# B10532021/Part-Aware_Measurement_for_3D_Pose_Estimation_and_Tracking

Hardware: AMD Instinct MI355X
Metric: multi-view frames/sec (end-to-end: HRNet-W48 2D pose + part-aware cross-view matching + DLT tracking) (higher is better)
Workload: dtype bf16 convs / f64 matching

## Files before the change

### part-aware_measurement_for_3d_pose_estimation_and_tracking_amd/csrc/pam_down.hip

```cpp
#include <hip/hip_runtime.h>
#include <stdint.h>
#include "../../include/pam.h"
#include "pam_resident.hpp"

namespace {

constexpr int PA = KStep48::PA, NST = KStep48::NST, WIMG = KStep48::WIMG;
constexpr int WPW = 6;
constexpr int BIASB = 2048;
constexpr int MTMAX = 3;
constexpr int D48_XSLOTS_MAX = (160 * 1024 - 2 * WIMG - BIASB) / PA;

struct D48Args {
    const uint16_t* in; const char* wpack; const float* bias; const uint16_t* res; uint16_t* out;
    int N, H, W, Ho, Wo, in_cs, out_cs, res_cs, relu, relu_from;
    int TR, TC, tiles_y, tiles_x, nitems, spw , xbytes;
    float inv_tc;
};

__device__ __attribute__((aligned(64))) const uint32_t g_d48_zero[16] = {0};

__global__ __launch_bounds__(512) void k_down48(D48Args a) {
    extern __shared__ __attribute__((aligned(1024))) char smem[];
    const int tid = threadIdx.x, lane = tid & 63, g = lane >> 4, l15 = lane & 15;
    const int wave = __builtin_amdgcn_readfirstlane(tid >> 6);
    const int bx = xcd_order(blockIdx.x, a.nitems);
    const int per_img = a.tiles_y * a.tiles_x;
    const int n = bx / per_img, trem = bx - n * per_img, tyi = trem / a.tiles_x, txi = trem - tyi * a.tiles_x;
    const int ty0 = tyi * a.TR, tx0 = txi * a.TC;
    const int NE = a.TC + 1, PWx = 2 * a.TC + 1, XR = 2 * a.TR + 1;
    const int slab0 = (int)blockIdx.y * a.spw;
    char* Xb = smem;
    float* bias_s = (float*)(smem + a.xbytes);
    char* Wb = smem + a.xbytes + BIASB;

    const float bv = (tid < a.spw * 48 && a.bias) ? a.bias[slab0 * 48 + tid] : 0.0f;
    const char* wsrc = a.wpack + (size_t)slab0 * WIMG + lane * 16;
    auto wdma = [&](int s) {
        char* dst = Wb + (s & 1) * WIMG;
#pragma unroll
        for (int k = 0; k < WPW; ++k) {
            const int p = min(wave + 8 * k, WIMG / 1024 - 1);
            __builtin_amdgcn_global_load_lds((glb_void*)(wsrc + (size_t)s * WIMG + p * 1024), (lds_void*)(dst + p * 1024), 16, 0, 0);
        }
    };
    wdma(0);
    {
        const int rowb = PWx * PA;
        const char* img = (const char*)a.in + (size_t)n * a.H * a.W * a.in_cs * 2;
        for (int k = 0; k * 1024 < rowb; ++k) {
            const int ob = k * 1024 + lane * 16;
            const int q = (int)(((unsigned)ob * 43691u) >> 22);
            const int rem = ob - q * PA;
            const int c = q < NE ? 2 * q : 2 * (q - NE) + 1;
            const int ix = 2 * tx0 - 1 + c;
            const bool okx = ob < rowb && (unsigned)ix < (unsigned)a.W;
            const long offx = (long)ix * a.in_cs * 2 + rem;
            if (ob < rowb) {
                for (int r = wave; r < XR; r += 8) {
                    const int iy = 2 * ty0 - 1 + r;
                    const bool ok = okx && (unsigned)iy < (unsigned)a.H;
                    const char* src = ok ? img + (size_t)iy * a.W * a.in_cs * 2 + offx : (const char*)g_d48_zero;
                    __builtin_amdgcn_global_load_lds((glb_void*)src, (lds_void*)(Xb + r * rowb + k * 1024), 16, 0, 0);
                }
            }
        }
    }
    if (tid < a.spw * 48) bias_s[tid] = bv;
    if (a.spw > 1) {
        wdma(1);
        asm volatile("s_waitcnt vmcnt(%0)" ::"n"(WPW) : "memory");
    } else {
        asm volatile("s_waitcnt vmcnt(0)" ::: "memory");
    }
    unsigned koff[NST];
#pragma unroll
    for (int st = 0; st < NST; ++st) {
        int k0 = 32 * st + 8 * g;
        if (k0 >= 432) k0 -= 16;
        const int t = k0 / 48, ch = k0 - 48 * t, ky = t / 3, kx = t - 3 * ky;
        koff[st] = (unsigned)((ky * PWx + (kx == 1 ? NE : (kx == 2 ? 1 : 0))) * PA + ch * 2);
    }
    const int npos = a.TR * a.TC;
    const int ntile = (npos + 15) >> 4, mt = (ntile - wave + 7) >> 3;
    const char* xl[MTMAX];
    long ooff[MTMAX];
#pragma unroll
    for (int i = 0; i < MTMAX; ++i) {
        const int m = (wave + 8 * i) * 16 + l15;
        const int r2 = fdiv_small(m, a.inv_tc), c2 = m - r2 * a.TC;
        const bool in_tile = m < npos;
        xl[i] = Xb + (in_tile ? (2 * r2 * PWx + c2) * PA : 0);
        const int oy = ty0 + r2, ox = tx0 + c2;
        ooff[i] = (in_tile && oy < a.Ho && ox < a.Wo) ? (long)(((size_t)n * a.Ho + oy) * a.Wo + ox) : -1;
    }
    const unsigned wlo = (unsigned)(l15 * 64 + ((g ^ KStep48::sigma(l15)) * 16));
    auto xaddr = [&](int i, int st) { return xl[i] + koff[st]; };

    asm volatile("s_barrier" ::: "memory");

    for (int s = 0; s < a.spw; ++s) {
        const int cb = (slab0 + s) * 48;
        u32x4 rq[MTMAX]; u32x2 rh[MTMAX];
        if (a.res) {
#pragma unroll
            for (int i = 0; i < MTMAX; ++i) {
                const uint16_t* rp = a.res + (ooff[i] >= 0 ? ooff[i] * a.res_cs + cb : 0);
                rq[i] = *(const u32x4*)(rp + 8 * g);
                rh[i] = *(const u32x2*)(rp + 32 + 4 * g);
            }
        }
        f32x4 acc[MTMAX][3];
        {
            const float* b = bias_s + s * 48;
            const f32x4 b0 = *(const f32x4*)(b + 8 * g), b1 = *(const f32x4*)(b + 8 * g + 4), b2 = *(const f32x4*)(b + 32 + 4 * g);
#pragma unroll
            for (int i = 0; i < MTMAX; ++i) { acc[i][0] = b0; acc[i][1] = b1; acc[i][2] = b2; }
        }
        const char* wl = Wb + (s & 1) * WIMG + wlo;
        if (mt >= 3) resident_pass<KStep48, 3>(acc, wl, xaddr, [](int) {});
        else if (mt == 2) resident_pass<KStep48, 2>(acc, wl, xaddr, [](int) {});
        else if (mt == 1) resident_pass<KStep48, 1>(acc, wl, xaddr, [](int) {});
        if (s + 1 < a.spw) {
            asm volatile("s_waitcnt vmcnt(0)" ::: "memory");
            asm volatile("s_barrier" ::: "memory");
            if (s + 2 < a.spw) wdma(s + 2);
        }
        const bool relu_lo = a.relu && cb + 8 * g >= a.relu_from, relu_hi = a.relu && cb + 32 + 4 * g >= a.relu_from;
#pragma unroll
        for (int i = 0; i < MTMAX; ++i) {
            if (i >= mt || ooff[i] < 0) continue;
            uint32_t ov[6];
#pragma unroll
            for (int j = 0; j < 3; ++j) {
                float v0 = acc[i][j][0], v1 = acc[i][j][1], v2 = acc[i][j][2], v3 = acc[i][j][3];
                if (a.res) {
                    const uint32_t r01 = j < 2 ? rq[i][2 * j] : rh[i][0], r23 = j < 2 ? rq[i][2 * j + 1] : rh[i][1];
                    v0 += bf16_lo(r01); v1 += bf16_hi(r01);
                    v2 += bf16_lo(r23); v3 += bf16_hi(r23);
                }
                ov[2 * j] = pack_bf16x2(v0, v1); ov[2 * j + 1] = pack_bf16x2(v2, v3);
                if (j < 2 ? relu_lo : relu_hi) { ov[2 * j] = relu_bf16x2(ov[2 * j]); ov[2 * j + 1] = relu_bf16x2(ov[2 * j + 1]); }
            }
            KStep48::store12(a.out + ooff[i] * a.out_cs + cb, g, ov);
        }
    }
}

bool d48_pick(int N, int Ho, int Wo, int nslab, int& TR, int& TC, int& G) {
    static thread_local int memo[8][7];
    static thread_local int memo_n = 0;
    for (int k = 0; k < 8 && k < memo_n; ++k)
        if (memo[k][0] == N && memo[k][1] == Ho && memo[k][2] == Wo && memo[k][3] == nslab) { TR = memo[k][4]; TC = memo[k][5]; G = memo[k][6]; return true; }
    long best = -1;
    for (int tr = 1; tr <= Ho; ++tr)
        for (int tc = 1; tc <= Wo; ++tc) {
            const int xs = (2 * tr + 1) * (2 * tc + 1), nt = (tr * tc + 15) / 16;
            if (xs > D48_XSLOTS_MAX || nt > 8 * MTMAX) continue;
            const long items = (long)N * ((Ho + tr - 1) / tr) * ((Wo + tc - 1) / tc);
            for (int gsz = 1; gsz <= nslab; ++gsz) {
                if (nslab % gsz) continue;
                const int spw = nslab / gsz;
                if (spw * 48 * 4 > BIASB) continue;
                const long fill = ((long)xs * PA + (long)spw * WIMG) / 24;
                const long mfma = (long)simd_tiles(nt, 0) * 3 * NST * 16 * spw;
                const long t = 5000 + (fill > mfma ? fill + mfma / 4 : mfma + fill / 4) + 500L * spw;
                const long wgs = items * gsz;
                const long cost = ((wgs + 255) / 256) * t * 4096 + wgs;
                if (best < 0 || cost < best) { best = cost; TR = tr; TC = tc; G = gsz; }
            }
        }
    if (best < 0) return false;
    int* m = memo[memo_n++ & 7];
    m[0] = N; m[1] = Ho; m[2] = Wo; m[3] = nslab; m[4] = TR; m[5] = TC; m[6] = G;
    return true;
}


struct DSArgs {
    const uint16_t* in; const uint16_t* wimg; const float* bias; uint16_t* out;
    int N, H, W, Ho, Wo, in_cs, Cout, TH, tiles_y, relu, relu_from;
    float inv_pwp, inv_wo;
};

template <int CIN, int NTW, int MT, int PMAX, int NBUF>
__global__ __launch_bounds__(512, 1) void k_down_s(DSArgs a) {
    constexpr int BN = 16 * NTW, NCHUNK = CIN / 32;
    constexpr int PIMG = PMAX * 64, WIMGS = 9 * BN * 64, BUF = PIMG + WIMGS;
    constexpr int PPW = PMAX / 64, WPIECES = WIMGS / 1024, WPWS = (WPIECES + 3) / 4, NPER = PPW + WPWS;
    static_assert(PMAX % 64 == 0 && WIMGS % 1024 == 0 && NPER * (NBUF - 1) <= 60 && NBUF >= 2 && NBUF <= 3, "ring shape");
    extern __shared__ __attribute__((aligned(1024))) char smem[];
    const int tid = threadIdx.x, lane = tid & 63, g = lane >> 4;
    const int wave = __builtin_amdgcn_readfirstlane(tid >> 6);
    const int ntiles = a.tiles_y * a.N;
    const int bx = xcd_order(blockIdx.x, ntiles);
    const int n = bx / a.tiles_y, ty0 = (bx - n * a.tiles_y) * a.TH;
    const int NEp = a.Wo + 1, PWp = 2 * a.Wo + 2, npatch = (2 * a.TH + 1) * PWp;
    const int npos = min(a.TH, a.Ho - ty0) * a.Wo;
    const int n0 = blockIdx.y * BN;

    if (wave >= 4) {
        const int lw = wave - 4;
        const char* psrc[PPW];
#pragma unroll
        for (int i = 0; i < PPW; ++i) {
            const int s = (lw + 4 * i) * 16 + (lane >> 2);
            const int gsrc = (lane & 3) ^ ((s >> 1) & 2);
            const int py = fdiv_small(s, a.inv_pwp), q = s - py * PWp;
            const int c = q < NEp ? 2 * q : 2 * (q - NEp) + 1;
            const int iy = 2 * ty0 - 1 + py, ix = c - 1;
            const bool ok = s < npatch && q <= 2 * a.Wo && (unsigned)iy < (unsigned)a.H && (unsigned)ix < (unsigned)a.W;
            psrc[i] = ok ? (const char*)a.in + (((size_t)n * a.H + iy) * a.W + ix) * (size_t)(a.in_cs * 2) + gsrc * 16 : (const char*)g_d48_zero;
        }
        const char* wsrc = (const char*)a.wimg + (size_t)blockIdx.y * NCHUNK * WIMGS + lane * 16;
        auto issue = [&](int c) {
            char* dst = smem + (size_t)((unsigned)c % (unsigned)NBUF) * BUF;
#pragma unroll
            for (int i = 0; i < (PPW > WPWS ? PPW : WPWS); ++i) {
                if (i < WPWS) {
                    const int j = min(lw + 4 * i, WPIECES - 1);
                    __builtin_amdgcn_global_load_lds((glb_void*)(wsrc + (size_t)c * WIMGS + j * 1024), (lds_void*)(dst + PIMG + j * 1024), 16, 0, 0);
                }
                if (i < PPW) {
                    const bool z = psrc[i] == (const char*)g_d48_zero;
                    __builtin_amdgcn_global_load_lds((glb_void*)(psrc[i] + (z ? 0 : c * 64)), (lds_void*)(dst + (lw + 4 * i) * 1024), 16, 0, 0);
                }
            }
        };
#pragma unroll
        for (int c = 0; c < NBUF - 1; ++c)
            if (c < NCHUNK) issue(c);
        for (int k = 0; k < NCHUNK; ++k) {
            const int fly = min(NCHUNK - 1 - k, NBUF - 2);
            dma_ring_wait<NPER, NBUF>(fly);
            asm volatile("s_barrier" ::: "memory");
            if (k + NBUF - 1 < NCHUNK) issue(k + NBUF - 1);
        }
        return;
    }

    f32x4 acc[MT][NTW];
    {
        f32x4 bias4[NTW];
#pragma unroll
        for (int j = 0; j < NTW; ++j) bias4[j] = a.bias ? *(const f32x4*)(a.bias + n0 + g * 4 * NTW + j * 4) : (f32x4){0.f, 0.f, 0.f, 0.f};
#pragma unroll
        for (int i = 0; i < MT; ++i)
#pragma unroll
            for (int j = 0; j < NTW; ++j) acc[i][j] = bias4[j];
    }
    unsigned aoff[MT][9];
    int opix[MT];
#pragma unroll
    for (int i = 0; i < MT; ++i) {
        const int m = (wave * MT + i) * 16 + (lane & 15);
        const int mm = m < npos ? m : 0;
        const int oy = fdiv_small(mm, a.inv_wo), ox = mm - oy * a.Wo;
        opix[i] = m < npos ? ((n * a.Ho + ty0 + oy) * a.Wo + ox) : -1;
#pragma unroll
        for (int t = 0; t < 9; ++t) {
            const int ky = t / 3, kx = t % 3;
            const int s = (2 * oy + ky) * PWp + ox + (kx == 1 ? NEp : (kx == 2 ? 1 : 0));
            aoff[i][t] = (unsigned)(s * 64 + ((g ^ ((s >> 1) & 2)) << 4));
        }
    }
    const unsigned woff = (unsigned)(PIMG + (lane & 15) * 64 + ((g ^ ((lane >> 1) & 2)) << 4));

    bf16x8 af[2][MT], bfr[2][NTW];
    auto ldfrag = [&](int k, int t, bf16x8* af_, bf16x8* bf_) {
        const char* buf = smem + (size_t)((unsigned)k % (unsigned)NBUF) * BUF;
#pragma unroll
        for (int j = 0; j < NTW; ++j) bf_[j] = *(const bf16x8*)(buf + woff + (t * BN + j * 16) * 64);
#pragma unroll
        for (int i = 0; i < MT; ++i) af_[i] = *(const bf16x8*)(buf + aoff[i][t]);
    };
    auto chunk = [&](int k, auto PARC) {
        constexpr int PAR = decltype(PARC)::value;
#pragma unroll
        for (int t = 0; t < 9; ++t) {
            const int cur = (t + PAR) & 1, nxt = cur ^ 1;
            if (t + 1 < 9) ldfrag(k, t + 1, af[nxt], bfr[nxt]);
            else if (k + 1 < NCHUNK) {
                __builtin_amdgcn_s_waitcnt(0xC07F);
                asm volatile("s_barrier" ::: "memory");
                ldfrag(k + 1, 0, af[nxt], bfr[nxt]);
            }
#pragma unroll
            for (int i = 0; i < MT; ++i)
#pragma unroll
                for (int j = 0; j < NTW; ++j)
                    acc[i][j] = __builtin_amdgcn_mfma_f32_16x16x32_bf16(__builtin_bit_cast(bf16x8_t, bfr[cur][j]),
                                                                       __builtin_bit_cast(bf16x8_t, af[cur][i]), acc[i][j], 0, 0, 0);
            spread<MT * NTW, MT + NTW>();
            __builtin_amdgcn_sched_barrier(0);
        }
    };
    asm volatile("s_barrier" ::: "memory");
    ldfrag(0, 0, af[0], bfr[0]);
    for (int k = 0; k < NCHUNK; k += 2) {
        chunk(k, std::integral_constant<int, 0>{});
        if (k + 1 < NCHUNK) chunk(k + 1, std::integral_constant<int, 1>{});
    }
#pragma unroll
    for (int i = 0; i < MT; ++i) {
        if (opix[i] < 0) continue;
        uint32_t ov[2 * NTW];
#pragma unroll
        for (int j = 0; j < NTW; ++j) {
            ov[2 * j] = pack_bf16x2(acc[i][j][0], acc[i][j][1]); ov[2 * j + 1] = pack_bf16x2(acc[i][j][2], acc[i][j][3]);
            if (a.relu && n0 + g * 4 * NTW + j * 4 >= a.relu_from) { ov[2 * j] = relu_bf16x2(ov[2 * j]); ov[2 * j + 1] = relu_bf16x2(ov[2 * j + 1]); }
        }
        row_store<NTW>(a.out + (size_t)opix[i] * a.Cout + n0 + g * 4 * NTW, g, ov);
    }
}

bool ds_pick(int Ho, int Wo, int Cin, int Cout, int& TH, int& bn) {
    if (Cin != 96 && Cin != 192) return false;
    bn = Cout % 64 == 0 ? 64 : (Cout % 48 == 0 ? 48 : 0);
    if (!bn) return false;
    const int PWp = 2 * Wo + 2;
    TH = 0;
    long best = 0;
    for (int t = Ho; t >= 1; --t) {
        if (t * Wo > 128 || (2 * t + 1) * PWp > 512) continue;
        const long cost = (Ho + t - 1) / t;
        if (TH == 0 || cost < best) { TH = t; best = cost; }
    }
    return TH >= 1;
}
template <int CIN, int NTW>
int launch_ds(hipStream_t s, const DSArgs& a) {
    constexpr int MT = 2, PMAX = 512, NBUF = 2;
    constexpr size_t lds = (size_t)NBUF * (PMAX * 64 + 9 * 16 * NTW * 64);
    static_assert(lds <= 160 * 1024, "LDS");
    if (!pam_max_dynamic_lds((const void*)k_down_s<CIN, NTW, MT, PMAX, NBUF>, (int)lds)) return PAM_E_HIP;
    pam_launch(k_down_s<CIN, NTW, MT, PMAX, NBUF>, dim3(a.tiles_y * a.N, a.Cout / (16 * NTW)), dim3(512), lds, s, a);
    return hipGetLastError() == hipSuccess ? PAM_OK : PAM_E_HIP;
}

}

extern "C" int pam_conv3x3s2_c48_tile(int N, int H, int W, int Cout, int32_t* out3) {
    if (N < 1 || H < 2 || W < 2 || Cout < 48 || Cout % 48 != 0 || !out3) return PAM_E_ARG;
    int tr = 0, tc = 0, gs = 0;
    if (!d48_pick(N, (H - 1) / 2 + 1, (W - 1) / 2 + 1, Cout / 48, tr, tc, gs)) return PAM_E_ARG;
    out3[0] = tr; out3[1] = tc; out3[2] = gs;
    return PAM_OK;
}

extern "C" int pam_conv3x3s2_c48_nhwc_bf16(void* stream, const void* in, int in_cstride, const void* wpack, const float* bias,
                                           const void* res, int res_cstride, void* out, int out_cstride, int N, int H, int W, int Cout,
                                           int relu, int relu_from, int tile_rows, int tile_cols, int slab_groups) {
    if (!in || !wpack || !out || N < 1 || H < 2 || W < 2 || Cout < 48 || Cout % 48 != 0) return PAM_E_ARG;
    if (in_cstride < 48 || in_cstride % 8 != 0 || out_cstride < Cout || out_cstride % 8 != 0 || relu_from < 0 || relu_from % 8 != 0) return PAM_E_ARG;
    if (res && (res_cstride < Cout || res_cstride % 8 != 0)) return PAM_E_ARG;
    D48Args a;
    a.in = (const uint16_t*)in; a.wpack = (const char*)wpack; a.bias = bias; a.res = (const uint16_t*)res; a.out = (uint16_t*)out;
    a.N = N; a.H = H; a.W = W; a.Ho = (H - 1) / 2 + 1; a.Wo = (W - 1) / 2 + 1;
    a.in_cs = in_cstride; a.out_cs = out_cstride; a.res_cs = res ? res_cstride : 0; a.relu = relu ? 1 : 0; a.relu_from = relu_from;
    if ((size_t)N * H * W * in_cstride * 2 >= (1ull << 40)) return PAM_E_ARG;
    const int nslab = Cout / 48;
    int G = slab_groups;
    if (tile_rows > 0 && tile_cols > 0) {
        a.TR = tile_rows; a.TC = tile_cols;
        if (G <= 0) G = 1;
    } else {
        int g2 = 1;
        if (!d48_pick(N, a.Ho, a.Wo, nslab, a.TR, a.TC, g2)) return PAM_E_ARG;
        if (G <= 0) G = g2;
    }
    if (a.TR > a.Ho) a.TR = a.Ho;
    if (a.TC > a.Wo) a.TC = a.Wo;
    if (nslab % G != 0) return PAM_E_ARG;
    a.spw = nslab / G;
    const int xs = (2 * a.TR + 1) * (2 * a.TC + 1);
    if (xs > D48_XSLOTS_MAX || (a.TR * a.TC + 15) / 16 > 8 * MTMAX || a.spw * 48 * 4 > BIASB) return PAM_E_ARG;
    a.xbytes = (xs * PA + 1023) / 1024 * 1024;
    a.tiles_y = (a.Ho + a.TR - 1) / a.TR; a.tiles_x = (a.Wo + a.TC - 1) / a.TC;
    const long long items = (long long)N * a.tiles_y * a.tiles_x;
    if (items >= (1ll << 30)) return PAM_E_ARG;
    a.nitems = (int)items;
    a.inv_tc = 1.0f / (float)a.TC;
    const size_t lds = (size_t)a.xbytes + BIASB + (size_t)(a.spw > 1 ? 2 : 1) * WIMG;
    if (!pam_max_dynamic_lds((const void*)k_down48, 160 * 1024)) return PAM_E_HIP;
    pam_launch(k_down48, dim3(a.nitems, G), dim3(512), lds, (hipStream_t)stream, a);
    return hipGetLastError() == hipSuccess ? PAM_OK : PAM_E_HIP;
}

extern "C" int pam_conv3x3s2_slab(int H, int W, int Cin, int Cout) {
    int th = 0, bn = 0;
    if (H < 2 || W < 2) return 0;
    return ds_pick((H - 1) / 2 + 1, (W - 1) / 2 + 1, Cin, Cout, th, bn) ? bn : 0;
}
extern "C" int pam_conv3x3s2_nhwc_bf16(void* stream, const void* in, int in_cstride, const void* w_img, const float* bias, void* out,
                                       int N, int H, int W, int Cin, int Cout, int relu, int relu_from) {
    if (!in || !w_img || !out || N < 1 || H < 2 || W < 2 || in_cstride < Cin || in_cstride % 8 != 0 || relu_from < 0 || relu_from % 16 != 0) return PAM_E_ARG;
    DSArgs a;
    a.in = (const uint16_t*)in; a.wimg = (const uint16_t*)w_img; a.bias = bias; a.out = (uint16_t*)out;
    a.N = N; a.H = H; a.W = W; a.Ho = (H - 1) / 2 + 1; a.Wo = (W - 1) / 2 + 1; a.in_cs = in_cstride; a.Cout = Cout;
    a.relu = relu ? 1 : 0; a.relu_from = relu_from;
    int bn = 0;
    if (!ds_pick(a.Ho, a.Wo, Cin, Cout, a.TH, bn)) return PAM_E_ARG;
    if ((size_t)N * a.Ho * a.Wo >= (1ull << 31) || (size_t)N * H * W * in_cstride * 2 >= (1ull << 40)) return PAM_E_ARG;
    a.tiles_y = (a.Ho + a.TH - 1) / a.TH;
    a.inv_pwp = 1.0f / (float)(2 * a.Wo + 2); a.inv_wo = 1.0f / (float)a.Wo;
    hipStream_t s = (hipStream_t)stream;
    switch (Cin * 10 + bn / 16) {
        case 964: return launch_ds<96, 4>(s, a);
        case 963: return launch_ds<96, 3>(s, a);
        case 1924: return launch_ds<192, 4>(s, a);
        case 1923: return launch_ds<192, 3>(s, a);
    }
    return PAM_E_ARG;
}
```

### part-aware_measurement_for_3d_pose_estimation_and_tracking_amd/engine.py

```python
import ctypes as C

import torch

from . import _lib
from .packing import down48_image, bf16_on, pointwise64_image, streamed_image


class ActivationArena(object):

    def __init__(self, device=None, half_bytes=None):
        self.half_bytes = half_bytes
        self.buf = torch.empty(2 * half_bytes, dtype=torch.uint8, device=device) if half_bytes else None
        self.half, self.off, self.peak = 1, 0, 0

    def epoch(self):
        self.half ^= 1
        self.off = 0

    def count(self, nbytes):
        self.off += (nbytes + 255) // 256 * 256
        self.peak = max(self.peak, self.off)

    def alloc(self, n, c, h, w):
        nbytes = 2 * n * c * h * w
        a = self.half * self.half_bytes + self.off
        self.count(nbytes)
        if self.off > self.half_bytes:
            raise _lib.PamError('activation arena too small: epoch needs > %d bytes' % self.half_bytes)
        return self.buf[a:a + nbytes].view(torch.bfloat16).as_strided((n, c, h, w), (h * w * c, 1, w * c, c))


class TileCfg(object):
    AUTO = -1
    CLASSIC = -2
    STATED_STREAMED = -3
    STATED_CLASSIC = -4
    C96_48 = -5
    C96_96 = -6
    GEN_STREAMED = -7
    SLAB32 = -8


def ptr(t):
    return C.c_void_p(t.data_ptr()) if t is not None else None


class ConvEngine(object):
    count = None
    prof = None
    arena = None
    _keep = None

    def _new(self, n, c, h, w, device):
        if self.arena is not None and device.type != 'meta':
            return self.arena.alloc(n, c, h, w)
        if self.arena is not None:
            self.arena.count(2 * n * c * h * w)
        y = torch.empty((n, c, h, w), dtype=torch.bfloat16, device=device, memory_format=torch.channels_last)
        if self._keep is not None:
            self._keep.append(y)
        return y

    def _cur(self, x):
        return C.c_void_p(torch.cuda.current_stream(x.device).cuda_stream)

    def _tally(self, x, nbytes, flops):
        if self.count is not None:
            self.count['bytes'] += nbytes; self.count['flops'] += flops; self.count['launches'] += 1
        return x.device.type == 'meta'

    def _run(self, x, name, call, nbytes, flops, family=None, sig=(), what=()):
        rc = call()
        if rc != 0:
            raise _lib.PamError('%s failed (%d)%s' % (name, rc, what[0] % tuple(what[1:]) if what else ''))
        if family is not None and self.prof is not None and x.device.type == 'cuda':
            if callable(family):
                family = family()
            self.prof.append(dict(family=family, sig=(family,) + tuple(sig), bytes=nbytes, flops=flops, fn=call))

    CONFIGS = {}
    config_name = None
    multi_stream = False
    flag_sync = True
    flags_on = False
    flag_host_err = None
    flag_max_us = 2000000
    flag_dev_void = None
    _flag_limit = None
    _flags = None

    def apply_config(self, name):
        for k, v in self.CONFIGS[name].items():
            setattr(self, k, v)
        self.config_name = name

    def flag_limit(self):
        if self._flag_limit is None:
            self._flag_limit = torch.tensor([int(self.flag_max_us)], dtype=torch.int32, device=self.device)
        return self._flag_limit

    def _epoch(self):
        if self.arena is not None:
            self.arena.epoch()

    def features(self, x8):
        self._keep = []
        return self._features(x8)

    pw64 = True
    slab32 = False
    gen_streamed = True
    tile_cfg = TileCfg.AUTO
    c96_slab = 0
    ACT = {None: 0, False: 0, True: 1, 'linear': 0, 'relu': 1, 'leaky': 2}

    @staticmethod
    def _cached(op, key, build):
        img = op._images.get(key)
        if img is None:
            img = op._images[key] = build()
        return img

    def conv(self, op, x, res=None, relu=False, res_after_act=False, relu_from=0):
        n, cin, h, w = x.shape
        T = TileCfg
        if (self.down48 and op.stride == 2 and op.kh == 3 and op.kw == 3 and op.pad == 1 and op.cin == 48 and op.cout % 48 == 0 and
                self.ACT[relu] <= 1 and not res_after_act and relu_from % 8 == 0):
            return self.conv_down48(op, x, res=res, relu=bool(self.ACT[relu]), relu_from=relu_from)
        if (self.down_s and op.stride == 2 and op.kh == 3 and op.kw == 3 and op.pad == 1 and op.cin in (96, 192) and res is None and
                self.ACT[relu] <= 1 and relu_from % 16 == 0 and self.tile_cfg == T.AUTO and
                (x.device.type == 'meta' or self.lib.pam_conv3x3s2_slab(h, w, cin, op.cout) > 0)):
            return self.conv_down_s(op, x, relu=bool(self.ACT[relu]), relu_from=relu_from)
        if (self.pw64 and op.kh == 1 and op.kw == 1 and op.stride == 1 and cin == 64 and op.cout == 64 and res is None and relu_from == 0 and
                self.ACT[relu] in (1, 2) and x.device.type != 'meta' and x.is_contiguous(memory_format=torch.channels_last) and n * h * w >= 65536):
            img = self._cached(op, 'pw64', lambda: bf16_on(pointwise64_image(op.w[:, :64].float().cpu()), op._device))
            y = self._new(n, 64, h, w, x.device)
            nbytes, flops = 2 * (x.numel() + y.numel() + 64 * 64) + 4 * 64, 2 * y.numel() * 64
            self._tally(x, nbytes, flops)
            self._run(x, 'pam_pointwise64_act_nhwc_bf16', lambda: self.lib.pam_pointwise64_act_nhwc_bf16(
                self._cur(x), ptr(x), ptr(img), ptr(op.bias), ptr(y), n * h * w, self.ACT[relu]), nbytes, flops)
            return y
        in_cs = cin if x.device.type == 'meta' else x.stride(3)
        assert cin == op.cin and (x.device.type == 'meta' or (x.stride(1) == 1 and x.stride(2) == w * in_cs and x.stride(0) == h * w * in_cs)), (x.shape, op.cin)
        ho = (h + 2 * op.pad - op.kh) // op.stride + 1
        wo = (w + 2 * op.pad - op.kw) // op.stride + 1
        y = self._new(n, op.cout, ho, wo, x.device)
        nbytes = 2 * (x.numel() + y.numel() + op.cout * op.kh * op.kw * op.cin + (y.numel() if res is not None else 0)) + 4 * op.cout
        flops = 2 * y.numel() * op.kh * op.kw * op.cin
        if self._tally(x, nbytes, flops):
            return y
        act = self.ACT[relu] | (4 if (res_after_act and res is not None) else 0)
        tile_cfg = T.CLASSIC if (self.tile_cfg == T.AUTO and act > 1) else self.tile_cfg
        wimg = None
        rows3x3 = (op.kh == 3 and op.kw == 3 and op.stride == 1 and op.pad == 1 and in_cs == cin and relu_from == 0 and
                   op._w_ohwi is not None)
        if tile_cfg == T.CLASSIC and self.gen_streamed and rows3x3 and self.lib.pam_conv3x3_layout_gen(h, w, cin, op.cout) > 0:
            bn = self.lib.pam_conv3x3_layout_gen(h, w, cin, op.cout)
            wimg = self._cached(op, ('gen', bn), lambda: streamed_image(op._w_ohwi, bn, op._device))
            tile_cfg = T.GEN_STREAMED
        if (wimg is None and self.slab32 and tile_cfg == T.AUTO and rows3x3 and cin in (192, 384) and
                self.lib.pam_conv3x3_layout_small(h, w, cin, op.cout) > 0):
            wimg = self._cached(op, ('s32', 32), lambda: streamed_image(op._w_ohwi, 32, op._device))
            tile_cfg = T.SLAB32
        if wimg is None:
            wimg = op.image(h, w, classic=(tile_cfg != T.AUTO), c96_slab=self.c96_slab) if (in_cs == cin and relu_from == 0) else None
        if tile_cfg == T.AUTO and wimg is not None and op._stem is None:
            if getattr(op, 'last_streamed', False):
                tile_cfg = {48: T.C96_48, 96: T.C96_96}.get(getattr(op, 'last_c96', 0), T.STATED_STREAMED)
            else:
                tile_cfg = T.STATED_CLASSIC

        def family():
            kind = self.lib.pam_conv_last_kernel()
            if kind == 4:
                return 'k_conv_stem %d->%d' % (3, op.cout)
            if kind in (1, 2):
                return '%s C=%d %dx%d' % ('k_conv3x3s' if kind == 2 else 'k_conv3x3', op.cin, h, w)
            return '%s %dx%d stride %d' % ('k_conv_gs' if kind == 3 else 'k_conv_igemm', op.kh, op.kw, op.stride)
        self._run(x, 'pam_conv2d_nhwc_bf16', lambda: self.lib.pam_conv2d_nhwc_bf16_ex(
            self._cur(x), ptr(x), ptr(op.w), ptr(wimg), ptr(op.bias), ptr(res), ptr(y),
            n, h, w, op.cin, op.cout, op.kh, op.kw, op.stride, op.pad, act, tile_cfg, in_cs, relu_from),
            nbytes, flops, family, (n, h, w, op.cin, op.cout, res is not None, in_cs, relu_from),
            what=(' for %s', (x.shape, op.cout, op.kh, op.stride)))
        return y

    down_s = True

    def conv_down_s(self, op, x, relu=False, relu_from=0):
        n, cin, h, w = x.shape
        in_cs = cin if x.device.type == 'meta' else x.stride(3)
        ho, wo = (h - 1) // 2 + 1, (w - 1) // 2 + 1
        y = self._new(n, op.cout, ho, wo, x.device)
        nbytes = 2 * (x.numel() + y.numel() + op.cout * 9 * cin) + 4 * op.cout
        flops = 2 * y.numel() * 9 * cin
        if self._tally(x, nbytes, flops):
            return y
        assert x.stride(1) == 1 and x.stride(2) == w * in_cs and x.stride(0) == h * w * in_cs, (x.shape, x.stride())
        bn = self.lib.pam_conv3x3s2_slab(h, w, cin, op.cout)
        img = self._cached(op, ('s2', bn), lambda: streamed_image(op.w[:, :9 * cin].float().cpu().reshape(op.cout, 3, 3, cin), bn, op._device))
        self._run(x, 'pam_conv3x3s2_nhwc_bf16', lambda: self.lib.pam_conv3x3s2_nhwc_bf16(
            self._cur(x), ptr(x), in_cs, ptr(img), ptr(op.bias), ptr(y), n, h, w, cin, op.cout, 1 if relu else 0, int(relu_from)),
            nbytes, flops, 'k_down_s 3x3 stride 2 C=%d %dx%d' % (cin, h, w), (n, h, w, op.cout, in_cs, relu_from),
            what=(' for %s -> %d', tuple(x.shape), op.cout))
        return y

    down48 = True
    d48_tile = None

    def conv_down48(self, op, x, res=None, relu=False, relu_from=0):
        n, cin, h, w = x.shape
        assert cin == 48 and op.cin == 48 and op.stride == 2 and op.kh == 3 and op.pad == 1
        in_cs = cin if x.device.type == 'meta' else x.stride(3)
        ho, wo = (h - 1) // 2 + 1, (w - 1) // 2 + 1
        y = self._new(n, op.cout, ho, wo, x.device)
        nbytes = 2 * (x.numel() + y.numel() + op.cout * 9 * 48 + (y.numel() if res is not None else 0)) + 4 * op.cout
        flops = 2 * y.numel() * 9 * 48
        if self._tally(x, nbytes, flops):
            return y
        assert x.stride(1) == 1 and x.stride(2) == w * in_cs and x.stride(0) == h * w * in_cs, (x.shape, x.stride())
        img = down48_image(op)
        t = self.d48_tile or (0, 0, 0)
        self._run(x, 'pam_conv3x3s2_c48_nhwc_bf16', lambda: self.lib.pam_conv3x3s2_c48_nhwc_bf16(
            self._cur(x), ptr(x), in_cs, ptr(img), ptr(op.bias), ptr(res), op.cout if res is not None else 0,
            ptr(y), op.cout, n, h, w, op.cout, 1 if relu else 0, int(relu_from), int(t[0]), int(t[1]), int(t[2])),
            nbytes, flops, 'k_down48 3x3 stride 2 C=48 %dx%d' % (h, w), (n, h, w, op.cout, res is not None, in_cs, relu_from),
            what=(' for %s -> %d', tuple(x.shape), op.cout))
        return y

    _bb2_tiles = {}
    b48_tile = None
    b96_tile = None

    def basic_block2(self, op, x, tile=None):
        n, c, h, w = x.shape
        assert c == op.c, (x.shape, op.c)
        y = self._new(n, c, h, w, x.device)
        nbytes, flops = 2 * (2 * x.numel() + 2 * 9 * c * c) + 8 * c, 2 * 2 * x.numel() * 9 * c
        if self._tally(x, nbytes, flops):
            return y
        assert x.is_contiguous(memory_format=torch.channels_last)
        if tile is None and c == 96 and self.b96_tile:
            tile = tuple(self.b96_tile)
        if tile is None and c == 48 and self.b48_tile:
            tile = tuple(self.b48_tile)
        if tile is None:
            tile = self._bb2_tiles.get((c, n, h, w))
            if tile is None:
                t2 = (C.c_int32 * 2)()
                if self.lib.pam_basic_block2_tile(c, n, h, w, t2) != 0:
                    raise _lib.PamError('no resident-weights block tile for %s' % (tuple(x.shape),))
                tile = self._bb2_tiles[(c, n, h, w)] = (int(t2[0]), int(t2[1]))
        self._run(x, 'pam_basic_block2_nhwc_bf16', lambda: self.lib.pam_basic_block2_nhwc_bf16(
            self._cur(x), ptr(x), ptr(op.wpack), ptr(y), n, h, w, c, tile[0], tile[1]),
            nbytes, flops, 'k_bblock2 C=%d' % c, (n, h, w, c) + tuple(tile), what=(' for %s tile %s', tuple(x.shape), tile))
        return y

    def pointwise64(self, op, x):
        n, c, h, w = x.shape
        assert c == 64
        y = self._new(n, c, h, w, x.device)
        nbytes, flops = 2 * (2 * x.numel() + 64 * 64) + 4 * 64, 2 * n * h * w * 64 * 64
        if self._tally(x, nbytes, flops):
            return y
        assert x.is_contiguous(memory_format=torch.channels_last)
        self._run(x, 'pam_pointwise64_relu_nhwc_bf16', lambda: self.lib.pam_pointwise64_relu_nhwc_bf16(
            self._cur(x), ptr(x), ptr(op.w), ptr(op.b), ptr(y), n * h * w), nbytes, flops, 'k_pw1 64->64 pointwise', (n, h, w))
        return y

    def stem_fused(self, op, x8):
        n, c, h, w = x8.shape
        assert c == 8
        h2, w2 = ((h - 1) // 2 + 1 - 1) // 2 + 1, ((w - 1) // 2 + 1 - 1) // 2 + 1
        x0 = self._new(n, 64, h2, w2, x8.device)
        y1 = self._new(n, 64, h2, w2, x8.device)
        h1, w1 = (h - 1) // 2 + 1, (w - 1) // 2 + 1
        nbytes = 2 * (x8.numel() + x0.numel() + y1.numel() + 64 * 72 + 64 * 576 + 64 * 64) + 4 * 192
        flops = 2 * n * (h1 * w1 * 64 * 72 + h2 * w2 * 64 * (576 + 64))
        if self._tally(x8, nbytes, flops):
            return x0, y1
        assert x8.is_contiguous(memory_format=torch.channels_last)
        self._run(x8, 'pam_stem_fused_nhwc_bf16', lambda: self.lib.pam_stem_fused_nhwc_bf16(
            self._cur(x8), ptr(x8), ptr(op.c1._stem), ptr(op.c1.bias), ptr(op.w2), ptr(op.b2), ptr(op.pw.w), ptr(op.pw.b),
            ptr(x0), ptr(y1), n, h, w), nbytes, flops, 'k_stem_fused stem + conv1 of layer1', (n, h, w), what=(' for %s', tuple(x8.shape)))
        return x0, y1

    def bottleneck_fused(self, op, y1, res=None, x0=None):
        n, c, h, w = y1.shape
        t = op.tail
        assert c == 64 and (res is None) != (x0 is None) and (x0 is None) == (t.S == 1)
        assert res is None or tuple(res.shape) == (n, 256, h, w)
        X = self._new(n, 256, h, w, y1.device)
        Y = self._new(n, 64, h, w, y1.device) if t.w1 is not None else None
        M = n * h * w
        side = res if res is not None else x0
        nbytes = 2 * (y1.numel() + side.numel() + X.numel() + (Y.numel() if Y is not None else 0) + 64 * 576 + t.S * 256 * 64 +
                      (64 * 256 if t.w1 is not None else 0)) + 4 * (64 + 256 + (64 if t.w1 is not None else 0))
        flops = 2 * M * (64 * 576 + t.S * 64 * 256 + (256 * 64 if t.w1 is not None else 0))
        if self._tally(y1, nbytes, flops):
            return X, Y
        for q in (y1, side):
            assert q.is_contiguous(memory_format=torch.channels_last)
        self._run(y1, 'pam_bottleneck_fused_nhwc_bf16', lambda: self.lib.pam_bottleneck_fused_nhwc_bf16(
            self._cur(y1), ptr(y1), ptr(x0), ptr(res), ptr(op.w2), ptr(op.b2), ptr(t.w3), ptr(t.b3), ptr(t.w1),
            ptr(t.b1), ptr(X), ptr(Y), n, h, w),
            nbytes, flops, 'k_bneck 3x3 + bottleneck tail', (n, h, w, t.S, t.w1 is not None), what=(' for %s', tuple(y1.shape)))
        return X, Y

    def bottleneck_tail(self, op, y2, x0=None, res=None, tile_cfg=0):
        n, c, h, w = y2.shape
        assert c == 64 and (x0 is None) == (op.S == 1), (y2.shape, op.S)
        X = self._new(n, 256, h, w, y2.device)
        Y = self._new(n, 64, h, w, y2.device) if op.w1 is not None else None
        M = n * h * w
        nbytes = 2 * (y2.numel() + (x0.numel() if x0 is not None else 0) + (res.numel() if res is not None else 0) + X.numel() +
                      (Y.numel() if Y is not None else 0) + op.S * 256 * 64 + (64 * 256 if op.w1 is not None else 0)) + 4 * (256 + (64 if op.w1 is not None else 0))
        flops = 2 * M * (op.S * 64 * 256 + (256 * 64 if op.w1 is not None else 0))
        if self._tally(y2, nbytes, flops):
            return X, Y
        for t in (y2, x0, res):
            assert t is None or t.is_contiguous(memory_format=torch.channels_last)
        self._run(y2, 'pam_bottleneck_tail_nhwc_bf16', lambda: self.lib.pam_bottleneck_tail_nhwc_bf16(
            self._cur(y2), ptr(y2), ptr(x0), ptr(res), ptr(op.w3), ptr(op.b3), ptr(op.w1), ptr(op.b1),
            ptr(X), ptr(Y), M, tile_cfg),
            nbytes, flops, 'k_pw2 bottleneck tail', (n, h, w, op.S, res is not None, op.w1 is not None), what=(' for %s', tuple(y2.shape)))
        return X, Y

    def upsample_add(self, base, terms, shifts, relu):
        n, c, h, w = base.shape
        y = self._new(n, c, h, w, base.device)
        nbytes = 2 * (2 * base.numel() + sum(t.numel() for t in terms))
        if self._tally(base, nbytes, 0):
            return y
        ptrs = (C.c_void_p * 3)(*[ptr(t) for t in terms] + [None] * (3 - len(terms)))
        sh = (C.c_int32 * 3)(*(list(shifts) + [0] * (3 - len(shifts))))
        cs = (C.c_int32 * 3)(*([t.stride(3) for t in terms] + [0] * (3 - len(terms))))
        self._run(base, 'pam_upsample_add_nhwc_bf16', lambda: self.lib.pam_upsample_add_nhwc_bf16_ex(
            self._cur(base), ptr(base), len(terms), ptrs, sh, cs, ptr(y), n, h, w, c, 1 if relu else 0),
            nbytes, 0, 'k_upsample_add', (n, h, w, c, len(terms)))
        return y

    def fuse_sum(self, op, base, plain, srcs, relu=True, tile=(0, 0), max_wg=0):
        n, c, h, w = base.shape
        assert c == op.c and len(srcs) == len(op.shifts) and len(plain) <= 2
        y = self._new(n, c, h, w, base.device)
        nbytes = 2 * (2 * base.numel() + sum(t.numel() for t in plain) + sum(t.numel() for t in srcs) + sum(c * cs for cs in op.chans)) + 4 * c * len(srcs)
        flops = sum(2 * t.shape[0] * t.shape[2] * t.shape[3] * t.shape[1] * c for t in srcs)
        if self._tally(base, nbytes, flops):
            return y
        for t, sh, cs in zip(srcs, op.shifts, op.chans):
            assert tuple(t.shape) == (n, cs, h >> sh, w >> sh) and t.is_contiguous(memory_format=torch.channels_last), (t.shape, base.shape, sh)
        pp = (C.c_void_p * 2)(*[ptr(t) for t in plain] + [None] * (2 - len(plain)))
        pcs = (C.c_int32 * 2)(*([t.stride(3) for t in plain] + [0] * (2 - len(plain))))
        sp = (C.c_void_p * len(srcs))(*[ptr(t) for t in srcs])
        self._run(base, 'pam_fuse_sum_nhwc_bf16', lambda: self.lib.pam_fuse_sum_nhwc_bf16(
            self._cur(base), ptr(base), len(plain), pp, pcs, len(srcs), sp, op.c_sh, op.c_ch, op.c_w, op.c_b, ptr(y),
            n, h, w, c, 1 if relu else 0, int(tile[0]), int(tile[1]), int(max_wg)),
            nbytes, flops, 'k_fuse_sum', (n, h, w, c, len(plain), len(srcs)), what=(' for %s', tuple(base.shape)))
        return y

    def upsample_concat(self, a, b):
        n, ca, h2, w2 = a.shape
        _, cb, h, w = b.shape
        assert h == 2 * h2 and w == 2 * w2 and b.shape[0] == n, (a.shape, b.shape)
        y = self._new(n, ca + cb, h, w, a.device)
        nbytes = 2 * (a.numel() + b.numel() + y.numel())
        if self._tally(a, nbytes, 0):
            return y
        self._run(a, 'pam_upsample_concat_nhwc_bf16', lambda: self.lib.pam_upsample_concat_nhwc_bf16(
            self._cur(a), ptr(a), ptr(b), ptr(y), n, h, w, ca, cb), nbytes, 0)
        return y

    def maxpool(self, x, size, stride):
        n, c, h, w = x.shape
        ho, wo = (h - 1) // stride + 1, (w - 1) // stride + 1
        y = self._new(n, c, ho, wo, x.device)
        nbytes = 2 * (x.numel() + y.numel())
        if self._tally(x, nbytes, 0):
            return y
        assert x.is_contiguous(memory_format=torch.channels_last), (x.shape, x.stride())
        self._run(x, 'pam_maxpool_nhwc_bf16', lambda: self.lib.pam_maxpool_nhwc_bf16(
            self._cur(x), ptr(x), ptr(y), n, h, w, c, int(size), int(stride)), nbytes, 0,
            what=(' for %s size %d stride %d', tuple(x.shape), size, stride))
        return y

    def spp(self, x, sizes):
        n, c, h, w = x.shape
        a, b, cc = [int(s) for s in sizes]
        y = self._new(n, 4 * c, h, w, x.device)
        nbytes = 2 * (x.numel() + y.numel())
        if self._tally(x, nbytes, 0):
            return y
        assert x.is_contiguous(memory_format=torch.channels_last), (x.shape, x.stride())
        self._run(x, 'pam_spp_concat_nhwc_bf16', lambda: self.lib.pam_spp_concat_nhwc_bf16(
            self._cur(x), ptr(x), ptr(y), n, h, w, c, a, b, cc), nbytes, 0, 'k_spp', (n, h, w, c, a, b, cc),
            what=(' for %s sizes %s', tuple(x.shape), (a, b, cc)))
        return y
```

Baseline: 458.1.

## Add warp-specialized row-staged stride-2 3x3 conv kernel for 256-channel inputs

Adds a new k_down_r kernel for 3x3 stride-2 convs with 256 input channels. Four producer waves stream per-(channel-chunk, kernel-row) patch and weight slices into a 3-deep LDS ring via global_load_lds, while four consumer waves run bf16 MFMAs with double-buffered fragments. The engine now routes cin=256 downsampling convs to this kernel instead of the generic path. It uses a new tile picker and weight image layout, so it depends on streamed_image producing a layout that matches the per-row staging.

```diff
diff --git a/part-aware_measurement_for_3d_pose_estimation_and_tracking_amd/csrc/pam_down.hip b/part-aware_measurement_for_3d_pose_estimation_and_tracking_amd/csrc/pam_down.hip
--- a/part-aware_measurement_for_3d_pose_estimation_and_tracking_amd/csrc/pam_down.hip
+++ b/part-aware_measurement_for_3d_pose_estimation_and_tracking_amd/csrc/pam_down.hip
@@ -338,6 +338,160 @@
     return hipGetLastError() == hipSuccess ? PAM_OK : PAM_E_HIP;
 }
 
+template <int CIN, int NTW, int MT, int PMAX, int NBUF>
+__global__ __launch_bounds__(512, 1) void k_down_r(DSArgs a) {
+    constexpr int BN = 16 * NTW, NSTAGE = 3 * (CIN / 32);
+    constexpr int PIMG = PMAX * 64, WIMGS = 3 * BN * 64, BUF = PIMG + WIMGS;
+    constexpr int PPW = PMAX / 64, WPIECES = WIMGS / 1024, WPWS = (WPIECES + 3) / 4, NPER = PPW + WPWS;
+    static_assert(PMAX % 64 == 0 && WIMGS % 1024 == 0 && NPER * (NBUF - 1) <= 60 && NBUF >= 2 && NBUF <= 3 && PPW <= 10 && NSTAGE % 2 == 0, "ring shape");
+    extern __shared__ __attribute__((aligned(1024))) char smem[];
+    const int tid = threadIdx.x, lane = tid & 63, g = lane >> 4;
+    const int wave = __builtin_amdgcn_readfirstlane(tid >> 6);
+    const int ntiles = a.tiles_y * a.N;
+    const int bx = xcd_order(blockIdx.x, ntiles);
+    const int n = bx / a.tiles_y, ty0 = (bx - n * a.tiles_y) * a.TH;
+    const int NEp = a.Wo + 1, PWp = 2 * a.Wo + 2, npatch = a.TH * PWp;
+    const int npos = min(a.TH, a.Ho - ty0) * a.Wo;
+    const int n0 = blockIdx.y * BN;
+
+    if (wave >= 4) {
+        const int lw = wave - 4;
+        const long rowb = (long)a.W * a.in_cs * 2;
+        const char* psrc[PPW];
+        unsigned okm = 0;
+#pragma unroll
+        for (int i = 0; i < PPW; ++i) {
+            const int s = (lw + 4 * i) * 16 + (lane >> 2);
+            const int gsrc = (lane & 3) ^ ((s >> 1) & 2);
+            const int r = fdiv_small(s, a.inv_pwp), q = s - r * PWp;
+            const int c = q < NEp ? 2 * q : 2 * (q - NEp) + 1;
+            const int iy0 = 2 * (ty0 + r) - 1, ix = c - 1;
+            const bool okx = s < npatch && q <= 2 * a.Wo && (unsigned)ix < (unsigned)a.W;
+#pragma unroll
+            for (int ky = 0; ky < 3; ++ky) okm |= (okx && (unsigned)(iy0 + ky) < (unsigned)a.H) ? 1u << (3 * i + ky) : 0u;
+            psrc[i] = (const char*)a.in + (((long)n * a.H + iy0) * a.W + ix) * (long)(a.in_cs * 2) + gsrc * 16;
+        }
+        const char* wsrc = (const char*)a.wimg + (size_t)blockIdx.y * NSTAGE * WIMGS + lane * 16;
+        auto issue = [&](int st) {
+            char* dst = smem + (size_t)((unsigned)st % (unsigned)NBUF) * BUF;
+            const int c = (int)((unsigned)st / 3u), ky = st - 3 * c;
+            const long poff = ky * rowb + c * 64;
+#pragma unroll
+            for (int i = 0; i < (PPW > WPWS ? PPW : WPWS); ++i) {
+                if (i < WPWS) {
+                    const int j = min(lw + 4 * i, WPIECES - 1);
+                    __builtin_amdgcn_global_load_lds((glb_void*)(wsrc + (size_t)st * WIMGS + j * 1024), (lds_void*)(dst + PIMG + j * 1024), 16, 0, 0);
+                }
+                if (i < PPW) {
+                    const char* src = ((okm >> (3 * i + ky)) & 1u) ? psrc[i] + poff : (const char*)g_d48_zero;
+                    __builtin_amdgcn_global_load_lds((glb_void*)src, (lds_void*)(dst + (lw + 4 * i) * 1024), 16, 0, 0);
+                }
+            }
+        };
+#pragma unroll
+        for (int st = 0; st < NBUF - 1; ++st) issue(st);
+        for (int k = 0; k < NSTAGE; ++k) {
+            const int fly = min(NSTAGE - 1 - k, NBUF - 2);
+            dma_ring_wait<NPER, NBUF>(fly);
+            asm volatile("s_barrier" ::: "memory");
+            if (k + NBUF - 1 < NSTAGE) issue(k + NBUF - 1);
+        }
+        return;
+    }
+
+    f32x4 acc[MT][NTW];
+    {
+        f32x4 bias4[NTW];
+#pragma unroll
+        for (int j = 0; j < NTW; ++j) bias4[j] = a.bias ? *(const f32x4*)(a.bias + n0 + g * 4 * NTW + j * 4) : (f32x4){0.f, 0.f, 0.f, 0.f};
+#pragma unroll
+        for (int i = 0; i < MT; ++i)
+#pragma unroll
+            for (int j = 0; j < NTW; ++j) acc[i][j] = bias4[j];
+    }
+    unsigned aoff[MT][3];
+    int opix[MT];
+#pragma unroll
+    for (int i = 0; i < MT; ++i) {
+        const int m = (wave * MT + i) * 16 + (lane & 15);
+        const int mm = m < npos ? m : 0;
+        const int oy = fdiv_small(mm, a.inv_wo), ox = mm - oy * a.Wo;
+        opix[i] = m < npos ? ((n * a.Ho + ty0 + oy) * a.Wo + ox) : -1;
+#pragma unroll
+        for (int kx = 0; kx < 3; ++kx) {
+            const int s = oy * PWp + ox + (kx == 1 ? NEp : (kx == 2 ? 1 : 0));
+            aoff[i][kx] = (unsigned)(s * 64 + ((g ^ ((s >> 1) & 2)) << 4));
+        }
+    }
+    const unsigned woff = (unsigned)(PIMG + (lane & 15) * 64 + ((g ^ ((lane >> 1) & 2)) << 4));
+
+    bf16x8 af[2][MT], bfr[2][NTW];
+    auto ldfrag = [&](int k, int t, bf16x8* af_, bf16x8* bf_) {
+        const char* buf = smem + (size_t)((unsigned)k % (unsigned)NBUF) * BUF;
+#pragma unroll
+        for (int j = 0; j < NTW; ++j) bf_[j] = *(const bf16x8*)(buf + woff + (t * BN + j * 16) * 64);
+#pragma unroll
+        for (int i = 0; i < MT; ++i) af_[i] = *(const bf16x8*)(buf + aoff[i][t]);
+    };
+    auto stage = [&](int k, auto PARC) {
+        constexpr int PAR = decltype(PARC)::value;
+#pragma unroll
+        for (int t = 0; t < 3; ++t) {
+            const int cur = (t + PAR) & 1, nxt = cur ^ 1;
+            if (t + 1 < 3) ldfrag(k, t + 1, af[nxt], bfr[nxt]);
+            else if (k + 1 < NSTAGE) {
+                __builtin_amdgcn_s_waitcnt(0xC07F);
+                asm volatile("s_barrier" ::: "memory");
+                ldfrag(k + 1, 0, af[nxt], bfr[nxt]);
+            }
+#pragma unroll
+            for (int i = 0; i < MT; ++i)
+#pragma unroll
+                for (int j = 0; j < NTW; ++j)
+                    acc[i][j] = __builtin_amdgcn_mfma_f32_16x16x32_bf16(__builtin_bit_cast(bf16x8_t, bfr[cur][j]),
+                                                                       __builtin_bit_cast(bf16x8_t, af[cur][i]), acc[i][j], 0, 0, 0);
+            spread<MT * NTW, MT + NTW>();
+            __builtin_amdgcn_sched_barrier(0);
+        }
+    };
+    asm volatile("s_barrier" ::: "memory");
+    ldfrag(0, 0, af[0], bfr[0]);
+    for (int k = 0; k < NSTAGE; k += 2) {
+        stage(k, std::integral_constant<int, 0>{});
+        stage(k + 1, std::integral_constant<int, 1>{});
+    }
+#pragma unroll
+    for (int i = 0; i < MT; ++i) {
+        if (opix[i] < 0) continue;
+        uint32_t ov[2 * NTW];
+#pragma unroll
+        for (int j = 0; j < NTW; ++j) {
+            ov[2 * j] = pack_bf16x2(acc[i][j][0], acc[i][j][1]); ov[2 * j + 1] = pack_bf16x2(acc[i][j][2], acc[i][j][3]);
+            if (a.relu && n0 + g * 4 * NTW + j * 4 >= a.relu_from) { ov[2 * j] = relu_bf16x2(ov[2 * j]); ov[2 * j + 1] = relu_bf16x2(ov[2 * j + 1]); }
+        }
+        row_store<NTW>(a.out + (size_t)opix[i] * a.Cout + n0 + g * 4 * NTW, g, ov);
+    }
+}
+
+constexpr int DR_MT = 4, DR_PMAX = 448;
+bool dr_pick(int Ho, int Wo, int Cout, int& TH, int& bn) {
+    bn = Cout % 96 == 0 ? 96 : (Cout % 48 == 0 ? 48 : 0);
+    if (!bn) return false;
+    const int PWp = 2 * Wo + 2;
+    TH = Ho < 64 * DR_MT / Wo ? Ho : 64 * DR_MT / Wo;
+    if (TH > DR_PMAX / PWp) TH = DR_PMAX / PWp;
+    return TH >= 1;
+}
+template <int CIN, int NTW>
+int launch_dr(hipStream_t s, const DSArgs& a) {
+    constexpr int NBUF = 3;
+    constexpr size_t lds = (size_t)NBUF * (DR_PMAX * 64 + 3 * 16 * NTW * 64);
+    static_assert(lds <= 160 * 1024, "LDS");
+    if (!pam_max_dynamic_lds((const void*)k_down_r<CIN, NTW, DR_MT, DR_PMAX, NBUF>, (int)lds)) return PAM_E_HIP;
+    pam_launch(k_down_r<CIN, NTW, DR_MT, DR_PMAX, NBUF>, dim3(a.tiles_y * a.N, a.Cout / (16 * NTW)), dim3(512), lds, s, a);
+    return hipGetLastError() == hipSuccess ? PAM_OK : PAM_E_HIP;
+}
+
 }
 
 extern "C" int pam_conv3x3s2_c48_tile(int N, int H, int W, int Cout, int32_t* out3) {
@@ -390,7 +544,8 @@
 extern "C" int pam_conv3x3s2_slab(int H, int W, int Cin, int Cout) {
     int th = 0, bn = 0;
     if (H < 2 || W < 2) return 0;
-    return ds_pick((H - 1) / 2 + 1, (W - 1) / 2 + 1, Cin, Cout, th, bn) ? bn : 0;
+    const int Ho = (H - 1) / 2 + 1, Wo = (W - 1) / 2 + 1;
+    return (Cin == 256 ? dr_pick(Ho, Wo, Cout, th, bn) : ds_pick(Ho, Wo, Cin, Cout, th, bn)) ? bn : 0;
 }
 extern "C" int pam_conv3x3s2_nhwc_bf16(void* stream, const void* in, int in_cstride, const void* w_img, const float* bias, void* out,
                                        int N, int H, int W, int Cin, int Cout, int relu, int relu_from) {
@@ -400,7 +555,7 @@
     a.N = N; a.H = H; a.W = W; a.Ho = (H - 1) / 2 + 1; a.Wo = (W - 1) / 2 + 1; a.in_cs = in_cstride; a.Cout = Cout;
     a.relu = relu ? 1 : 0; a.relu_from = relu_from;
     int bn = 0;
-    if (!ds_pick(a.Ho, a.Wo, Cin, Cout, a.TH, bn)) return PAM_E_ARG;
+    if (!(Cin == 256 ? dr_pick(a.Ho, a.Wo, Cout, a.TH, bn) : ds_pick(a.Ho, a.Wo, Cin, Cout, a.TH, bn))) return PAM_E_ARG;
     if ((size_t)N * a.Ho * a.Wo >= (1ull << 31) || (size_t)N * H * W * in_cstride * 2 >= (1ull << 40)) return PAM_E_ARG;
     a.tiles_y = (a.Ho + a.TH - 1) / a.TH;
     a.inv_pwp = 1.0f / (float)(2 * a.Wo + 2); a.inv_wo = 1.0f / (float)a.Wo;
@@ -410,6 +565,8 @@
         case 963: return launch_ds<96, 3>(s, a);
         case 1924: return launch_ds<192, 4>(s, a);
         case 1923: return launch_ds<192, 3>(s, a);
+        case 2566: return launch_dr<256, 6>(s, a);
+        case 2563: return launch_dr<256, 3>(s, a);
     }
     return PAM_E_ARG;
 }
diff --git a/part-aware_measurement_for_3d_pose_estimation_and_tracking_amd/engine.py b/part-aware_measurement_for_3d_pose_estimation_and_tracking_amd/engine.py
--- a/part-aware_measurement_for_3d_pose_estimation_and_tracking_amd/engine.py
+++ b/part-aware_measurement_for_3d_pose_estimation_and_tracking_amd/engine.py
@@ -127,7 +127,7 @@
         if (self.down48 and op.stride == 2 and op.kh == 3 and op.kw == 3 and op.pad == 1 and op.cin == 48 and op.cout % 48 == 0 and
                 self.ACT[relu] <= 1 and not res_after_act and relu_from % 8 == 0):
             return self.conv_down48(op, x, res=res, relu=bool(self.ACT[relu]), relu_from=relu_from)
-        if (self.down_s and op.stride == 2 and op.kh == 3 and op.kw == 3 and op.pad == 1 and op.cin in (96, 192) and res is None and
+        if (self.down_s and op.stride == 2 and op.kh == 3 and op.kw == 3 and op.pad == 1 and op.cin in (96, 192, 256) and res is None and
                 self.ACT[relu] <= 1 and relu_from % 16 == 0 and self.tile_cfg == T.AUTO and
                 (x.device.type == 'meta' or self.lib.pam_conv3x3s2_slab(h, w, cin, op.cout) > 0)):
             return self.conv_down_s(op, x, relu=bool(self.ACT[relu]), relu_from=relu_from)
@@ -200,7 +200,7 @@
         img = self._cached(op, ('s2', bn), lambda: streamed_image(op.w[:, :9 * cin].float().cpu().reshape(op.cout, 3, 3, cin), bn, op._device))
         self._run(x, 'pam_conv3x3s2_nhwc_bf16', lambda: self.lib.pam_conv3x3s2_nhwc_bf16(
             self._cur(x), ptr(x), in_cs, ptr(img), ptr(op.bias), ptr(y), n, h, w, cin, op.cout, 1 if relu else 0, int(relu_from)),
-            nbytes, flops, 'k_down_s 3x3 stride 2 C=%d %dx%d' % (cin, h, w), (n, h, w, op.cout, in_cs, relu_from),
+            nbytes, flops, '%s 3x3 stride 2 C=%d %dx%d' % ('k_down_r' if cin == 256 else 'k_down_s', cin, h, w), (n, h, w, op.cout, in_cs, relu_from),
             what=(' for %s -> %d', tuple(x.shape), op.cout))
         return y
 
```

New measurement: 461.4, median of 4. No clear change (+0.7%).
